# mmp/pbrt-v4

Hardware: AMD Instinct MI355X
Metric: Msamples/sec (whole node), 1920x1080 at fixed spp (higher is better)
Workload: dtype f32; 1 GPU; San Miguel 1080p 256spp (BASELINE.json configs[2]) on the sanmiguel-like stand-in at the SURVEY 8(d) spec: 10001008 unique triangles in 2000 meshes, 60 % of them in 200 object-instance definitions (two-level BVH), 10 % alpha-cut, 1k^2 image textures, diffuse / coated diffuse / dielectric / conductor, sun + 2k^2 image sky + 500 emitters, maxdepth 5, zsobol; step = 1 sample index x 1920x1080; spp=321, samples_per_pass=64, partition=single GPU

## Files before the change

### pbrt-v4_amd/csrc/common/wf_kernels.h

```cpp
#pragma once

#include "wf_bxdf.h"
#include "wf_camera.h"
#include "wf_lights.h"
#include "wf_media.h"
#include "wf_bssrdf.h"
#include "wf_hair.h"
#include "wf_measured.h"

namespace wf {

struct alignas(16) F4 { float x, y, z, w; };
struct alignas(16) I4 { int32_t x, y, z, w; };
struct alignas(8) I2 { int32_t x, y; };
WF_HD F4 toF4(S4 s) { return F4{s[0], s[1], s[2], s[3]}; }
WF_HD S4 toS4(F4 f) { return S4{{f.x, f.y, f.z, f.w}}; }

enum {
    CNT_RAY0 = 0, CNT_RAY1 = 1, CNT_ESCAPED = 2, CNT_HITLIGHT = 3, CNT_SHADOW = 4, CNT_MAT0 = 5,
    CNT_MEDIUM_SAMPLE = CNT_MAT0 + WF_MAT_NTYPES, CNT_MEDIUM_SCATTER, CNT_MIX, CNT_RETRACE, CNT_BSSRDF, CNT_SSS, CNT_CURSOR, CNT_TR0, CNT_TR1,
    CNT_RETRACE_HEAD, CNT_WAVES_DONE,
    CNT_CURSOR_SHADOW,
    CNT_MEDIUM_ROUTE,
    CNT_DEFER, CNT_DEFER_SHADOW,
    CNT_CURSOR_MEDIUM,
    CNT_COUNT
};
constexpr int CNT_STRIDE = 64;
static_assert(CNT_COUNT <= 32, "k_reset takes the counters to zero as a 32-bit mask");
enum { RAYFLAG_SPECULAR_BOUNCE = 1, RAYFLAG_ANY_NONSPECULAR = 2 };

struct RayQueueV {
    F4 *o;
    F4 *d;
    F4 *beta, *r_u, *r_l;
    F4 *ctx0;
    F4 *ctx1;
    F4 *ctx2;
    I4 *meta;
};
struct ShadowQueueV {
    F4 *o;
    F4 *d;
    F4 *Ld, *r_u, *r_l;
    int32_t *medium;
};
struct BssrdfItem {
    F4 beta, r_u;
    V3 p; float etaScale;
    V3 wo; int depth;
    N3 n; int pixelIndex;
    N3 ns; int material;
    V3 dpdus; int mediumInside;
    V2 uv; int mediumOutside; int pad;
};
struct SubsurfaceItem {
    V3 p0, p1;
    int depth, material;
    TabulatedBSSRDF bssrdf;
    F4 beta, r_u;
    float reservoirPDF;
    P3i pi;
    N3 n, ns;
    V3 dpdu, dpdv, dpdus, dpdvs;
    int mediumInside, mediumOutside;
    float etaScale;
    int pixelIndex;
};
struct WorkState {
    int maxQueueSize;
    int pixelsPerPass, samplesPerPass;
    int slotStride = 0;
    int drainEpoch = 0;
    int stripRank, stripCount, stripHeight, localRows;
    float *filterWeight;
    I2 *pPixel;
    F4 *lambda, *lambdaPdf, *L, *cameraRayWeight;
    F4 *samples0;
// ... 1525 lines not shown
```

### pbrt-v4_amd/csrc/hip/wf_backend.hip

```cpp
#include <hip/hip_runtime.h>
#include <climits>
#include <cstdio>
#include <cstring>
#include <algorithm>
#include <map>
#include <string>
#include <type_traits>
#include <utility>
#include <vector>

#pragma clang attribute push(__attribute__((uninitialized)), apply_to = variable(is_local))
#include "../common/wf_kernels.h"
#include "../common/wf_kat.h"
#pragma clang attribute pop
#include "wf_traverse.h"
#include "wf_plan.h"
#include "wf_film_develop.h"

using namespace wf;
using namespace wf::planning;

#define HIPCHK(call)                                                                                        \
    do {                                                                                                    \
        hipError_t e_ = (call);                                                                             \
        if (e_ != hipSuccess) return fail((int)e_, "%s failed: %s (%s:%d)", #call, hipGetErrorString(e_), __FILE__, __LINE__); \
    } while (0)

constexpr int BLOCK = 256;
constexpr int MAX_GRID = 256 * 8;

struct SpillArea { int *base; int rows; int *dbg; };

using ClosestWalkFn = void (*)(const SceneView, WorkState, FastBVH, int, SpillArea, int *, int, const int *);
using ShadowWalkFn = void (*)(const SceneView, WorkState, FastBVH, SpillArea, int *, int, const int *);
using TrTraceFn = void (*)(const SceneView, WorkState, FastBVH, int, SpillArea);
using TraceClosestFn = void (*)(const SceneView, FastBVH, int, const float *, wf_hit_record *, SpillArea);
using TraceAnyFn = void (*)(const SceneView, FastBVH, int, const float *, int32_t *, SpillArea);
struct WalkKernels {
    ClosestWalkFn closest = nullptr;
    ShadowWalkFn shadow = nullptr;
    ClosestWalkFn closestGen = nullptr;
    ShadowWalkFn shadowGen = nullptr;
    int grid = 1024, gridShadow = 1024, gridGen = 1024, gridShadowGen = 1024;
    TrTraceFn trTrace = nullptr;
    TraceClosestFn traceClosest = nullptr;
    TraceAnyFn traceAny = nullptr;
    TraceClosestFn traceClosest8 = nullptr;
    TraceAnyFn traceAny8 = nullptr;
};


struct wf_ctx {
    int device = 0;
    hipStream_t stream = nullptr;
    std::vector<void *> allocs;
    SceneView svHost{};
    const SceneView *svDev = nullptr;
    WorkState ws{};
    int maxQueueSize = 0;
    int *stackSpill = nullptr;
    int *dbgWords = nullptr;
    SpillArea spillArea() const { return SpillArea{stackSpill, plan.spillRows, dbgWords}; }
    FastBVH fast{};
    hipStream_t stream2 = nullptr;
    hipEvent_t evFork = nullptr, evJoin = nullptr;
    bool retracePending = false, deferJoin = false;
    hipStream_t stream3 = nullptr;
    hipEvent_t evShadowFork = nullptr, evShadowJoin = nullptr;
    int frameOverlap = 1;
    bool shadowPending = false;
    int *stackSpill2 = nullptr;
    int32_t *deferQShadow = nullptr;
    bool samplesShaded = true;
    bool cursorDirty[2] = {false, false};
    ScenePlan plan;
    WalkKernels walk;
    struct TrScratch {
        F4 *o = nullptr, *d = nullptr, *lambdaPdf = nullptr;
        float *pathTime = nullptr;
        F4 *trO = nullptr, *trD = nullptr, *trT = nullptr, *trRu = nullptr, *trRl = nullptr, *hit = nullptr;
        I4 *trRng = nullptr;
        int32_t *trQ[2] = {nullptr, nullptr}, *hitInst = nullptr;
        int32_t *counters = nullptr;
        size_t capacity = 0;
        struct Slot { void **p; size_t elem; bool wavefront; };
        std::vector<Slot> slots() {
            return {{(void **)&o, sizeof(F4), false}, {(void **)&d, sizeof(F4), false}, {(void **)&lambdaPdf, sizeof(F4), false}, {(void **)&pathTime, sizeof(float), false},
                    {(void **)&trO, sizeof(F4), true}, {(void **)&trD, sizeof(F4), true}, {(void **)&trT, sizeof(F4), true}, {(void **)&trRu, sizeof(F4), true},
                    {(void **)&trRl, sizeof(F4), true}, {(void **)&hit, sizeof(F4), true}, {(void **)&trRng, sizeof(I4), true},
                    {(void **)&trQ[0], sizeof(int32_t), true}, {(void **)&trQ[1], sizeof(int32_t), true}, {(void **)&hitInst, sizeof(int32_t), true}};
        }
    } trScratch;
    int32_t *probeCursor = nullptr;
// ... 480 lines not shown
        }
        const bool valid = idx < n;
        RayWalk w;
        w.node = NODE_NONE;
        w.prim = -1;
        w.route = 0;
        w.tMax = 0;
        w.b0 = w.b1 = w.b2 = 0;
        w.inst = w.curInst = -1;
        if (valid) {
            V3 o, d;
            float tMax;
            fetch(idx, &o, &d, &tMax);
            WalkInit(bvh, w, o, d, tMax);
            if constexpr (INST || GEN > 0) StoreWorldRay(o, d);
            st.reset();
        }
        while (__any(w.node != NODE_NONE)) {
            while (WalkDescend<INST, ANY>(w)) {
                if (w.node >= 0) {
                    U4 nd[QNODE_U4];
                    FetchNode(bvh, w.node, nd);
                    InteriorStep<!ANY>(bvh, w, st, nd);
                }
            }
            LeafPhase<ANY, GEN, INST>(sv, bvh, w, st, fetch, idx);
        }
        if constexpr (!ANY && RetraceInline(GenBase(GEN))) {
            static_assert(ANY || !GenDefer(GEN), "the inline re-walk's `w.route = rh.route` would drop WALK_DEFER: the handing-over variants must walk with BatchTraceRefill");
            if (valid && WalkAmbiguous(w)) {
                V3 o, d;
                float t0;
                fetch(idx, &o, &d, &t0);
                const float tB = __builtin_fminf(2 * WalkBound(bvh, WalkT(w)) - WalkT(w), t0);
                const RefHit rh = RetraceRefOrder<GenBase(GEN), GenAnim(GEN)>(bvh.sv, o.x, o.y, o.z, d.x, d.y, d.z, tB, st.spill, st.spillStride, st.rows, st.dbg, GenAnim(GEN) ? g_time[threadIdx.x] : 0.f);
                w.prim = rh.prim; w.inst = rh.inst; w.route = rh.route;
                w.tMax = rh.t; w.b0 = rh.b0; w.b1 = rh.b1; w.b2 = rh.b2;
            }
        }
        finish(idx, valid, w);
    }
}

#ifndef WF_REFILL_AT
#define WF_REFILL_AT 40
#endif
#ifndef WF_GUIDED_CHUNK
#define WF_GUIDED_CHUNK 6
#endif
#ifndef WF_GUIDED_DIV
#define WF_GUIDED_DIV 4
#endif
template <bool ANY, int GEN, bool INST = false, bool DRAIN = false, typename Fetch, typename Finish>
__device__ inline void BatchTraceRefill(const SceneView &sv, const FastBVH &bvh, int n, LdsStackT &st, Fetch fetch, Finish finish, int *cursor = nullptr, int chunk = 4,
                                        int workBlocks = 0) {
    if (workBlocks <= 0) workBlocks = (int)gridDim.x;
    if (n < 2 * workBlocks * TBLOCK) cursor = nullptr;
    if (cursor && st.dbg && threadIdx.x == 0 && blockIdx.x == 0) atomicOr(st.dbg + 3, 1);
    const int lane = threadIdx.x & 63;
    const int waveId = (blockIdx.x * TBLOCK + threadIdx.x) >> 6, nWaves = (workBlocks * TBLOCK) >> 6;
    const int runRays = cursor ? 64 * chunk : 64;
    int next = 0, end = 0, staticJ = 0;
    int lastB = 0;
    bool exhausted = false;
    int idx = -1;
#if WF_WALK_ZERO
    RayWalk w{};
#else
    RayWalk w;
#endif
    w.node = NODE_NONE;
    w.prim = -1;
    w.route = 0;
    w.tMax = 0;
    w.b0 = w.b1 = w.b2 = 0;
    w.inst = w.curInst = -1;
    WalkStats ws_;
    auto retire = [&]() {
        finish(idx, true, w);
        idx = -1;
    };
    while (true) {
        const unsigned long long act = __ballot(w.node != NODE_NONE);
        const int nAct = __popcll(act);
        if (nAct <= WF_REFILL_AT && !exhausted) {
            const bool idle = w.node == NODE_NONE;
            if (idle && idx >= 0) retire();
            const int need = 64 - nAct;
            const int rank = __popcll(~act & ((1ull << lane) - 1ull));
            int served = 0;
            while (served < need) {
                if (next >= end) {
                    int b;
                    int rr = runRays;
                    if (cursor) {
#if WF_GUIDED_CHUNK
                        if constexpr (ANY && GenBase(GEN) <= 1) { int c = (n - lastB) / (nWaves * 64 * WF_GUIDED_DIV); c = c < 1 ? 1 : (c > WF_GUIDED_CHUNK ? WF_GUIDED_CHUNK : c); rr = 64 * c; }
#endif
                        b = 0;
                        if (lane == 0) b = atomicAdd(cursor, rr);
                        b = __builtin_amdgcn_readfirstlane(b);
                        lastB = b < n ? b : n;
                    } else {
                        b = (staticJ * nWaves + waveId) * 64;
                        ++staticJ;
                    }
                    next = b;
                    end = b + rr < n ? b + rr : n;
                    if (next >= n) { exhausted = true; break; }
                }
                const int take = need - served < end - next ? need - served : end - next;
                if (idle && rank >= served && rank < served + take) idx = next + (rank - served);
                next += take;
                served += take;
            }
            ws_.add(3, idle && idx >= 0);
            if (idle && idx >= 0) {
                V3 o, d;
                float tMax;
                fetch(idx, &o, &d, &tMax);
                WalkInit(bvh, w, o, d, tMax);
                if constexpr (INST || GEN > 0) StoreWorldRay(o, d);
                st.reset();
            }
            if (exhausted && !__any(w.node != NODE_NONE)) break;
        } else if (nAct == 0) break;
        while (WalkDescend<INST, ANY>(w)) {
            ws_.add(0, w.node >= 0);
            if (w.node >= 0) {
                U4 nd[QNODE_U4];
                FetchNode(bvh, w.node, nd);
                InteriorStep<!ANY>(bvh, w, st, nd);
            }
        }
        if constexpr (WF_WALK_STATS != 0) ws_.add(1, w.node < 0 && w.node != NODE_NONE && !(INST && AtTransition(w.node)));
        const int ranT = LeafPhase<ANY, GEN, INST>(sv, bvh, w, st, fetch, idx);
        if constexpr (WF_WALK_STATS != 0) { if (ranT) { ws_.c[4] += 1; ws_.c[5] += (unsigned long long)ranT; } }
    }
    ws_.flush(st.dbg, ANY ? 1 : 0);
    if (idx >= 0) retire();
}
template <bool ANY, int GEN, bool INST, bool DRAIN = false, typename Fetch, typename Finish>
__device__ inline void TraceQueue(const SceneView &sv, const FastBVH &bvh, int n, LdsStackT &st, Fetch fetch, Finish finish, int *cursor = nullptr, int chunk = 4,
                                  int workBlocks = 0) {
    if constexpr (ANY || DRAIN || !RetraceInline(GenBase(GEN))) BatchTraceRefill<ANY, GEN, INST, DRAIN>(sv, bvh, n, st, fetch, finish, cursor, chunk, workBlocks);
    else BatchTrace<ANY, GEN, INST>(sv, bvh, n, st, fetch, finish, cursor, chunk);
}
#ifndef WF_SERVICE_BLOCKS
#define WF_SERVICE_BLOCKS 16
#endif
__device__ inline int ServiceBlocks() { return (int)gridDim.x >= 8 * WF_SERVICE_BLOCKS ? WF_SERVICE_BLOCKS : 0; }
template <int GEN, bool INST, bool ANIM = false>
__device__ inline void DrainRetrace(const SceneView &sv, const WorkState &ws, const FastBVH &bvh, int cur, LdsStackT &st, bool service) {
    int *cnt = ws.counters + CNT_RETRACE * CNT_STRIDE, *head = ws.counters + CNT_RETRACE_HEAD * CNT_STRIDE, *done = ws.counters + CNT_WAVES_DONE * CNT_STRIDE;
    const int lane = threadIdx.x & 63;
    const int totalWaves = (int)gridDim.x * (TBLOCK / 64), workerWaves = ((int)gridDim.x - ServiceBlocks()) * (TBLOCK / 64);
    const RayQueueV &q = ws.rq[cur];
    auto takeSome = [&]() -> bool {
        int base = 0, take = 0;
        if (lane == 0) {
            while (true) {
                const int h = __hip_atomic_load(head, __ATOMIC_RELAXED, __HIP_MEMORY_SCOPE_AGENT), c = __hip_atomic_load(cnt, __ATOMIC_RELAXED, __HIP_MEMORY_SCOPE_AGENT);
                if (h >= c) break;
                const int t = c - h < 64 ? c - h : 64;
                if (atomicCAS(head, h, h + t) == h) { base = h; take = t; break; }
            }
        }
        base = __builtin_amdgcn_readfirstlane(base);
        take = __builtin_amdgcn_readfirstlane(take);
        if (take == 0) return false;
        if (lane < take) {
            unsigned long long e;
            while ((uint32_t)((e = __hip_atomic_load(&ws.retraceQ64[base + lane], __ATOMIC_ACQUIRE, __HIP_MEMORY_SCOPE_AGENT)) >> 32) != (uint32_t)ws.drainEpoch) {}
            const int i = (int)(uint32_t)(e & 0xffffffffull);
            const float tB = BitsToFloat((uint32_t)__hip_atomic_load(&ws.retraceQ[base + lane], __ATOMIC_RELAXED, __HIP_MEMORY_SCOPE_AGENT));
            const F4 o = q.o[i], d = q.d[i];
            RefHit rh;
            int tries = 0;
            do { rh = RetraceRefOrder<GEN, ANIM>(bvh.sv, o.x, o.y, o.z, d.x, d.y, d.z, tB, st.spill, st.spillStride, st.rows, st.dbg, o.w); } while (rh.prim < 0 && ++tries < 4);
            if (st.dbg && tries) { atomicAdd(st.dbg + 5, tries); if (rh.prim < 0) atomicOr(st.dbg + 6, 1); }
            if (st.dbg) {
                const bool badIndex = i < 0 || i >= ws.counters[(CNT_RAY0 + cur) * CNT_STRIDE];
                const bool badHit = rh.prim >= 0 && !(rh.t <= tB);
                const bool badTag = (uint32_t)(__hip_atomic_load(&ws.retraceQ64[base + lane], __ATOMIC_RELAXED, __HIP_MEMORY_SCOPE_AGENT) >> 32) != (uint32_t)ws.drainEpoch;
                if (badIndex || badHit || badTag) atomicOr(st.dbg + 6, 2);
            }
            ws.routeCode[i] = rh.route;
            ws.hit[i] = F4{BitsToFloat((uint32_t)rh.prim), rh.b0, rh.b1, rh.b2};
            if (INST) ws.hitInst[i] = rh.prim >= 0 ? rh.inst : -1;
            if (sv.haveMedia) ws.hitT[i] = rh.prim >= 0 ? rh.t : WF_INFINITY;
        }
        return true;
    };
    auto signOff = [&]() -> int {
        int prev = 0;
        if (lane == 0) { __threadfence(); prev = atomicAdd(done, 1); }
        return __builtin_amdgcn_readfirstlane(prev);
    };
    bool last;
    if (!service) {
        while (takeSome()) {}
        last = signOff() == totalWaves - 1;
        if (last) while (takeSome()) {}
    } else {
        while (true) {
            if (takeSome()) continue;
            int dn = 0;
            if (lane == 0) dn = __hip_atomic_load(done, __ATOMIC_RELAXED, __HIP_MEMORY_SCOPE_AGENT);
            dn = __builtin_amdgcn_readfirstlane(dn);
            if (dn >= workerWaves) {
                if (takeSome()) continue;
                break;
            }
            __builtin_amdgcn_s_sleep(64);
        }
        last = signOff() == totalWaves - 1;
    }
    if (last && lane == 0) {
        __hip_atomic_store(head, 0, __ATOMIC_RELAXED, __HIP_MEMORY_SCOPE_AGENT);
        __hip_atomic_store(cnt, 0, __ATOMIC_RELAXED, __HIP_MEMORY_SCOPE_AGENT);
        __hip_atomic_store(done, 0, __ATOMIC_RELAXED, __HIP_MEMORY_SCOPE_AGENT);
    }
}

constexpr uint32_t ROUTE_SKIP = 0x80000000u;
constexpr int TWavesFor(int gen, int triangleWaves) { return gen == 3 ? 2 : triangleWaves; }
template <int GENX, bool INST = false>
__global__ void __launch_bounds__(TBLOCK, TWavesFor(GenBase(GENX), INST ? WF_TWAVES_INST : WF_TWAVES_CLOSEST)) k_closest_fast(const SceneView svArg, WorkState ws, FastBVH bvh, int cur, SpillArea sp, int *cursor = nullptr, int chunk = 4, const int *list = nullptr) {
    constexpr int GEN = GenBase(GENX);
    const SceneView &sv = SvOf<false>(svArg);
    const int n = list ? ws.counters[(CNT_DEFER) * CNT_STRIDE] : ws.counters[(CNT_RAY0 + cur) * CNT_STRIDE];
    const int gtid = blockIdx.x * TBLOCK + threadIdx.x, stride = gridDim.x * TBLOCK;
    LdsStackT st{sp.base + gtid, stride, 0, 0, sp.rows, sp.dbg};
    const RayQueueV q = ws.rq[cur];
    constexpr bool DRAIN = RetraceInline(GEN);
    const int workBlocks = DRAIN ? (int)gridDim.x - ServiceBlocks() : (int)gridDim.x;
    if (DRAIN && (int)blockIdx.x >= workBlocks) { DrainRetrace<GEN, INST, GenAnim(GENX)>(sv, ws, bvh, cur, st, true); return; }
    TraceQueue<false, GENX, INST, DRAIN>(
        sv, bvh, n, st,
        [&](int i0, V3 *o, V3 *d, float *tMax) {
            const int i = list ? list[i0] : i0;
            F4 o4 = q.o[i], d4 = q.d[i];
            *o = V3{o4.x, o4.y, o4.z}; *d = V3{d4.x, d4.y, d4.z}; *tMax = WF_INFINITY;
            if constexpr (GenAnim(GENX)) {
                g_time[threadIdx.x] = o4.w;
                ws.pathTime[q.meta[i].x] = o4.w;
            }
        },
        [&](int i0, bool valid, const RayWalk &w) {
            const int i = (list && valid) ? list[i0] : i0;
            if constexpr (GenDefer(GENX))
                if (valid && (w.route & WALK_DEFER)) {
                    ws.deferQ[QueueAlloc(&ws.counters[(CNT_DEFER) * CNT_STRIDE])] = i;
                    ws.routeCode[i] = ROUTE_SKIP;
                    return;
                }
            const bool amb = valid && WalkAmbiguous(w);
            if (amb) {
                const int slot = atomicAdd(&ws.counters[(CNT_RETRACE) * CNT_STRIDE], 1);
                const float bound = 2 * WalkBound(bvh, WalkT(w)) - WalkT(w);
                if constexpr (DRAIN) {
                    if (sp.dbg) atomicAdd(sp.dbg + 4, 1);
                    __hip_atomic_store(&ws.retraceQ[slot], (int)FloatToBits(bound), __ATOMIC_RELAXED, __HIP_MEMORY_SCOPE_AGENT);
                    __hip_atomic_store(&ws.retraceQ64[slot], (unsigned long long)(uint32_t)i | ((unsigned long long)(uint32_t)ws.drainEpoch << 32), __ATOMIC_RELEASE, __HIP_MEMORY_SCOPE_AGENT);
                    return;
                } else {
                    ws.retraceQ[slot] = i;
                    ws.hit[i] = F4{0, bound, 0, 0};
                }
            }
            if (!valid) return;
            ws.routeCode[i] = amb ? ROUTE_SKIP : (uint32_t)w.route;
            if (amb) return;
            ws.hit[i] = F4{BitsToFloat((uint32_t)w.prim), w.b0, w.b1, w.b2};
            if (INST) ws.hitInst[i] = w.prim >= 0 ? w.inst : -1;
            if (sv.haveMedia) ws.hitT[i] = w.prim >= 0 ? WalkT(w) : WF_INFINITY;
        }, cursor, chunk, workBlocks);
    if constexpr (DRAIN) DrainRetrace<GEN, INST, GenAnim(GENX)>(sv, ws, bvh, cur, st, false);
}
constexpr int RBLOCK = 1024;
constexpr int RouteBlock(bool anim) { return anim ? BLOCK : RBLOCK; }
template <bool GENERAL, bool ANIM = false>
__global__ void __launch_bounds__(RouteBlock(ANIM)) k_route_hits(const SceneView svArg, WorkState ws, int cur) {
    constexpr int RB = RouteBlock(ANIM);
    const SceneView &sv = SvOf<true>(svArg);
    const int n = ws.counters[(CNT_RAY0 + cur) * CNT_STRIDE];
    for (int base = blockIdx.x * RB; base < n; base += gridDim.x * RB) {
        const int i = base + threadIdx.x;
        bool valid = i < n;
        uint32_t route = 0;
        F4 h{0, 0, 0, 0};
        int inst = -1;
        float tHit = 0;
        if (valid) {
            route = ws.routeCode[i];
            if (route & ROUTE_SKIP) valid = false;
            else {
                h = ws.hit[i];
                if (sv.nInstances > 0) inst = ws.hitInst[i];
                if (sv.haveMedia) tHit = ws.hitT[i];
            }
        }
        KRouteHitBlock<GENERAL, ANIM>(sv, ws, cur, i, valid, (int)FloatToBits(h.x), route, tHit, h.y, h.z, h.w, inst);
    }
}
__global__ void __launch_bounds__(BLOCK) k_closest_retrace(const SceneView sv, WorkState ws, int cur, int *stackSpill) {
    const int n = ws.counters[(CNT_RETRACE) * CNT_STRIDE];
    const int gtid = blockIdx.x * BLOCK + threadIdx.x, stride = gridDim.x * BLOCK;
    LdsStack st{stackSpill + gtid, stride, 0};
    for (int qi = gtid; qi < n; qi += stride) {
        const int i = ws.retraceQ[qi];
        F4 o = ws.rq[cur].o[i], d = ws.rq[cur].d[i];
        ClosestHit ch;
        st.n = 0;
        bool found = BVHIntersectClosest(sv, V3{o.x, o.y, o.z}, V3{d.x, d.y, d.z}, ws.hit[i].y, st, &ch);
        KAfterClosestHit(sv, ws, cur, i, found, ch.prim, ch.inst, ch.h.t, ch.h.b0, ch.h.b1, ch.h.b2);
    }
}
__global__ void __launch_bounds__(BLOCK) k_subsurface_probe(const SceneView sv, WorkState ws) {
    const int n = ws.counters[(CNT_BSSRDF) * CNT_STRIDE];
    for (int i = blockIdx.x * BLOCK + threadIdx.x; i < n; i += gridDim.x * BLOCK) KSubsurfaceProbe(sv, ws, i);
}
template <bool ANIM>
__global__ void __launch_bounds__(BLOCK) k_intersect_one_random(const SceneView sv, WorkState ws, int *stackSpill) {
    const int n = ws.counters[(CNT_SSS) * CNT_STRIDE];
    const int gtid = blockIdx.x * BLOCK + threadIdx.x, stride = gridDim.x * BLOCK;
    LdsStack st{stackSpill + gtid, stride, 0};
    for (int i = gtid; i < n; i += stride) KIntersectOneRandom<ANIM>(sv, ws, i, st);
}
template <bool ANIM>
__global__ void __launch_bounds__(BLOCK) k_trace_one_random(const SceneView sv, int n, const float *segs, int segStride, const int32_t *material, const float *times,
// ... 458 lines not shown

struct ClosestWalk { using Fn = ClosestWalkFn; template <int G, bool I> static Fn of() { return k_closest_fast<G, I>; } };
struct ShadowWalk { using Fn = ShadowWalkFn; template <int G, bool I> static Fn of() { return k_shadow_fast<G, I>; } };
struct TrTraceWalk { using Fn = TrTraceFn; template <int G, bool I> static Fn of() { return k_tr_trace<G, I>; } };
struct TraceClosestWalk { using Fn = TraceClosestFn; template <int G, bool I> static Fn of() { return k_trace_closest_fast<G, I>; } };
struct TraceAnyWalk { using Fn = TraceAnyFn; template <int G, bool I> static Fn of() { return k_trace_any_fast<G, I>; } };
struct TraceClosestWalk8 { using Fn = TraceClosestFn; template <int G, bool I> static Fn of() { return k_trace_closest_fast<G, I, 8>; } };
struct TraceAnyWalk8 { using Fn = TraceAnyFn; template <int G, bool I> static Fn of() { return k_trace_any_fast<G, I, 8>; } };
template <typename K, bool INST, int G>
static typename K::Fn WalkVariant() {
    if constexpr (GenAnim(G) && !INST) return nullptr;
    else return K::template of<G, INST>();
}
template <typename K, int... G>
static typename K::Fn PickWalk(int genx, bool inst, std::integer_sequence<int, G...>) {
    typename K::Fn f = nullptr;
    ((genx == G ? (void)(f = inst ? WalkVariant<K, true, G>() : WalkVariant<K, false, G>()) : (void)0), ...);
    return f;
}
static int PickWalkKernels(wf_ctx *ctx) {
    using QueueWalks = std::integer_sequence<int, 0, 1, 2, 3, GenX(0, true, false), GenX(1, true, false), GenX(0, false, true), GenX(1, false, true)>;
    const bool inst = ctx->svHost.nInstances > 0;
    const int gen = ctx->plan.genMode;
    const int first = ctx->plan.deferGeneral ? GenX(ctx->plan.genTri, true, false) : GenX(gen, false, ctx->plan.animFast);
    WalkKernels k;
    k.closest = PickWalk<ClosestWalk>(first, inst, QueueWalks{});
    k.shadow = PickWalk<ShadowWalk>(first, inst, QueueWalks{});
    if (ctx->plan.deferGeneral) {
        k.closestGen = PickWalk<ClosestWalk>(gen, inst, QueueWalks{});
        k.shadowGen = PickWalk<ShadowWalk>(gen, inst, QueueWalks{});
    }
    k.traceClosest = PickWalk<TraceClosestWalk>(gen, inst, std::integer_sequence<int, 0, 1, 2, 3>{});
    k.traceAny = PickWalk<TraceAnyWalk>(gen, inst, std::integer_sequence<int, 0, 1, 2, 3>{});
    {
        using TimedWalks = std::integer_sequence<int, 0, 1, 2, 3, GenX(0, false, true), GenX(1, false, true)>;
        k.traceClosest8 = PickWalk<TraceClosestWalk8>(GenX(gen, false, ctx->plan.animFast), inst, TimedWalks{});
        k.traceAny8 = PickWalk<TraceAnyWalk8>(GenX(gen, false, ctx->plan.animFast), inst, TimedWalks{});
    }
    if (RetraceInline(gen)) k.trTrace = PickWalk<TrTraceWalk>(GenX(gen, false, ctx->plan.animFast), inst, std::integer_sequence<int, 0, 1, GenX(0, false, true), GenX(1, false, true)>{});
    if (!k.closest || !k.shadow || !k.traceClosest || !k.traceAny || !k.traceClosest8 || !k.traceAny8 || (ctx->plan.deferGeneral && (!k.closestGen || !k.shadowGen)) || (RetraceInline(gen) && !k.trTrace))
        return fail(-1, "no walk kernel for this scene (genMode %d, genTri %d, two-class %d, animated %d, instances %d)", gen, ctx->plan.genTri, (int)ctx->plan.deferGeneral, (int)ctx->plan.animFast, (int)inst);
    hipDeviceProp_t prop;
    HIPCHK(hipGetDeviceProperties(&prop, ctx->device));
    const int maxG = MAX_GRID * BLOCK / TBLOCK;
    auto residentGrid = [&](auto kernel, int *out) {
        int perCU = 0;
        HIPCHK(hipOccupancyMaxActiveBlocksPerMultiprocessor(&perCU, (const void *)kernel, TBLOCK, 0));
        *out = std::min(maxG, std::max(1, perCU) * prop.multiProcessorCount);
        return 0;
    };
    int e;
    if ((e = residentGrid(k.closest, &k.grid)) || (e = residentGrid(k.shadow, &k.gridShadow))) return e;
    if (ctx->plan.deferGeneral && ((e = residentGrid(k.closestGen, &k.gridGen)) || (e = residentGrid(k.shadowGen, &k.gridShadowGen)))) return e;
    ctx->walk = k;
    return 0;
}

extern "C" {

int wf_abi_version(void) { return WF_ABI_VERSION; }

constexpr int SCRATCH_PRIME_WORDS = 896;
__global__ void k_scratch_prime(int *out, int n) {
    volatile int buf[SCRATCH_PRIME_WORDS];
    for (int i = 0; i < n; ++i) buf[(i * 131) % SCRATCH_PRIME_WORDS] = i;
    out[threadIdx.x] = buf[(n * 7) % SCRATCH_PRIME_WORDS];
}
static void DestroyCtx(wf_ctx *ctx) {
    (void)hipSetDevice(ctx->device);
    if (ctx->stream) (void)hipStreamSynchronize(ctx->stream);
    if (ctx->stream3) (void)hipStreamSynchronize(ctx->stream3);
    for (void *p : ctx->allocs) (void)hipFree(p);
    for (const wf_ctx::TrScratch::Slot &sl : ctx->trScratch.slots())
        if (*sl.p) (void)hipFree(*sl.p);
    if (ctx->trScratch.counters) (void)hipFree(ctx->trScratch.counters);
    for (auto &e : ctx->events) { (void)hipEventDestroy(e.a); (void)hipEventDestroy(e.b); }
    for (auto e : ctx->eventPool) (void)hipEventDestroy(e);
    if (ctx->stream) (void)hipStreamDestroy(ctx->stream);
    if (ctx->stream2) (void)hipStreamDestroy(ctx->stream2);
    if (ctx->stream3) (void)hipStreamDestroy(ctx->stream3);
    if (ctx->evShadowFork) (void)hipEventDestroy(ctx->evShadowFork);
    if (ctx->evShadowJoin) (void)hipEventDestroy(ctx->evShadowJoin);
    if (ctx->evFork) (void)hipEventDestroy(ctx->evFork);
    if (ctx->evJoin) (void)hipEventDestroy(ctx->evJoin);
    delete ctx;
}
static int InitCtx(wf_ctx *c, const Switches &sw) {
    HIPCHK(hipStreamCreateWithFlags(&c->stream, hipStreamNonBlocking));
    HIPCHK(hipStreamCreateWithFlags(&c->stream2, hipStreamNonBlocking));
    HIPCHK(hipStreamCreateWithFlags(&c->stream3, hipStreamNonBlocking));
    HIPCHK(hipEventCreateWithFlags(&c->evFork, hipEventDisableTiming));
    HIPCHK(hipEventCreateWithFlags(&c->evJoin, hipEventDisableTiming));
    HIPCHK(hipEventCreateWithFlags(&c->evShadowFork, hipEventDisableTiming));
    HIPCHK(hipEventCreateWithFlags(&c->evShadowJoin, hipEventDisableTiming));
    c->frameOverlap = sw.frameOverlap;
    c->samplesShaded = sw.samplesShaded;
    c->traceLaunch = sw.traceLaunch;
    if (sw.scratchPrime) {
        DeviceScratch tmp(c->stream);
        int *out = nullptr;
        if (int e = tmp.alloc(&out, (size_t)64)) return e;
        hipLaunchKernelGGL(k_scratch_prime, dim3(1), dim3(64), 0, c->stream, out, 8);
        hipLaunchKernelGGL(k_scratch_prime, dim3(1), dim3(64), 0, c->stream2, out, 8);
        hipLaunchKernelGGL(k_scratch_prime, dim3(1), dim3(64), 0, c->stream3, out, 8);
        HIPCHK(hipStreamSynchronize(c->stream));
        HIPCHK(hipStreamSynchronize(c->stream2));
        HIPCHK(hipStreamSynchronize(c->stream3));
    }
    return 0;
}
int wf_ctx_create(int device, wf_ctx **out) {
    if (!out) return fail(-1, "null out");
    int ndev = 0;
    HIPCHK(hipGetDeviceCount(&ndev));
    if (ndev <= 0) return fail(-1, "no HIP device visible: libwfhip has no CPU fallback");
    if (device < 0 || device >= ndev) return fail(-1, "device %d out of range (0..%d)", device, ndev - 1);
    HIPCHK(hipSetDevice(device));
    wf_ctx *c = new wf_ctx();
    c->device = device;
    if (int e = InitCtx(c, Switches::FromEnv())) { DestroyCtx(c); return e; }
    *out = c;
    return 0;
}

int wf_ctx_destroy(wf_ctx *ctx) {
    if (ctx) DestroyCtx(ctx);
    return 0;
}

int wf_sync(wf_ctx *ctx) {
    if (!ctx) return fail(-1, "null context");
    useDevice(ctx);
    HIPCHK(hipStreamSynchronize(ctx->stream));
    HIPCHK(hipGetLastError());
    if (ctx->dbgWords) {
        int overflow = 0;
        HIPCHK(hipMemcpy(&overflow, ctx->dbgWords + 1, sizeof(int), hipMemcpyDeviceToHost));
        if (overflow) return fail(-1, "traversal stack overflow: a walk needed more than %d + %d node-stack entries (results are incomplete)", TSTACK, ctx->plan.spillRows);
        int unresolved = 0;
        HIPCHK(hipMemcpy(&unresolved, ctx->dbgWords + 6, sizeof(int), hipMemcpyDeviceToHost));
        if (unresolved & 1) return fail(-1, "a near-tie re-walk found no hit where the production walk had one (results are incomplete)");
        if (unresolved & 2) return fail(-1, "a near-tie queue entry failed its validation (ray index, bound or launch tag): results are incomplete");
        int fatal = 0;
        HIPCHK(hipMemcpy(&fatal, ctx->dbgWords + 7, sizeof(int), hipMemcpyDeviceToHost));
        if (fatal) return fail(-1, "%s", FatalMessage(fatal));
        if (getenv("WF_DEBUG_DRAIN")) {
            int h[8];
            HIPCHK(hipMemcpy(h, ctx->dbgWords, sizeof(h), hipMemcpyDeviceToHost));
            fprintf(stderr, "[drain] spilled %d, re-walks %d, pushes %d, repeated re-walks %d, unresolved %d\n", h[0], h[2], h[4], h[5], h[6]);
#if WF_WALK_STATS
            unsigned long long c[16];
            HIPCHK(hipMemcpy(c, ctx->dbgWords + 8, sizeof(c), hipMemcpyDeviceToHost));
            const char *ph[4] = {"interior", "leaf", "transition", "refill"};
            for (int k = 0; k < 2; ++k)
                for (int q = 0; q < 4; ++q)
                    fprintf(stderr, "[walk stats] %s %-26s wave iterations %llu, lanes %llu (%.1f per iteration)\n", k ? "any-hit" : "closest", ph[q], c[k * 8 + 2 * q], c[k * 8 + 2 * q + 1],
                            c[k * 8 + 2 * q] ? (double)c[k * 8 + 2 * q + 1] / (double)c[k * 8 + 2 * q] : 0.0);
#endif
        }
    }
    return 0;
}
int wf_debug_counters(wf_ctx *ctx, uint64_t out[4], int reset) {
    if (!ctx || !ctx->sceneLoaded || !out) return fail(-1, "wf_debug_counters: no scene uploaded");
    int h[4] = {0, 0, 0, 0};
    HIPCHK(hipStreamSynchronize(ctx->stream));
    HIPCHK(hipMemcpy(h, ctx->dbgWords, sizeof(h), hipMemcpyDeviceToHost));
    for (int i = 0; i < 4; ++i) out[i] = (uint64_t)(unsigned)h[i];
    if (reset) HIPCHK(hipMemset(ctx->dbgWords, 0, sizeof(h)));
    return 0;
}
void *wf_stream(wf_ctx *ctx) { return ctx ? (void *)ctx->stream : nullptr; }

static int UploadTables(wf_ctx *ctx, const wf_scene_desc *d, const Switches &sw) {
    SceneView &sv = ctx->svHost;
    const ScenePlan &plan = ctx->plan;
    int e = 0;
    if ((e = devUpload(ctx, &sv.P, d->P, (size_t)3 * d->n_vertices))) return e;
    if ((e = devUpload(ctx, &sv.N, d->N, (size_t)3 * d->n_vertices))) return e;
    if ((e = devUpload(ctx, &sv.UV, d->UV, (size_t)2 * d->n_vertices))) return e;
    if (d->n_tangents > 0 && (e = devUpload(ctx, &sv.S, d->S, (size_t)3 * d->n_tangents))) return e;
    if ((e = devUpload(ctx, &sv.triIndices, d->tri_indices, (size_t)3 * d->n_triangles))) return e;
    if ((e = devUpload(ctx, &sv.triMesh, d->tri_mesh, (size_t)d->n_triangles + d->n_quadrics))) return e;
    sv.shadeTris = nullptr;
    if (d->n_triangles > 0 && sw.shadeTris) {
        std::vector<ShadeTri> st((size_t)d->n_triangles);
        for (size_t t = 0; t < (size_t)d->n_triangles; ++t) {
            const int32_t *ix = d->tri_indices + 3 * t;
            const int flags = d->meshes[d->tri_mesh[t]].flags;
            ShadeTri r{};
            for (int k = 0; k < 3; ++k) {
                for (int a = 0; a < 3; ++a) r.p[3 * k + a] = d->P[3 * (size_t)ix[k] + a];
                if ((flags & WF_MESH_HAS_N) && d->N) for (int a = 0; a < 3; ++a) r.n[3 * k + a] = d->N[3 * (size_t)ix[k] + a];
                if ((flags & WF_MESH_HAS_UV) && d->UV) for (int a = 0; a < 2; ++a) r.uv[2 * k + a] = d->UV[2 * (size_t)ix[k] + a];
            }
// ... 269 lines not shown
        int planes = 0;
        for (int m = 1; m < WF_MAT_NTYPES; ++m) if (ctx->plan.matPresent[m]) planes = std::max(planes, NeePlanes(m));
        if (planes > 0 && (e = devAlloc(ctx, &ws.neeRec, n * (size_t)planes))) return e;
    }
    if ((e = devAlloc(ctx, &ws.routeCode, n))) return e;
    ctx->maxQueueSize = max_queue_size;
    ctx->queuesAllocated = true;
    return 0;
}

int wf_set_pass_samples(wf_ctx *ctx, int sample_step, int n_samples) {
    if (int e = checkReady(ctx)) return e;
    if (n_samples < 1 || n_samples > ctx->ws.samplesPerPass) return fail(-1, "n_samples %d outside 1..%d", n_samples, ctx->ws.samplesPerPass);
    if (sample_step < 1) return fail(-1, "sample_step must be >= 1");
    ctx->passStep = sample_step;
    ctx->passSamples = n_samples;
    ctx->ws.slotStride = ctx->pixelMajor ? n_samples : 0;
    return 0;
}

int wf_set_strips(wf_ctx *ctx, int rank, int count, int height, int *local_rows) {
    if (!ctx || !ctx->sceneLoaded) return fail(-1, "no scene uploaded");
    useDevice(ctx);
    if (count < 1 || rank < 0 || rank >= count || height < 1) return fail(-1, "wf_set_strips: rank %d of %d, height %d", rank, count, height);
    int rows = 0;
    for (int y = 0; y < ctx->H; ++y) rows += (y / height) % count == rank;
    ctx->ws.stripRank = rank; ctx->ws.stripCount = count; ctx->ws.stripHeight = height; ctx->ws.localRows = count > 1 ? rows : ctx->H;
    if (local_rows) *local_rows = ctx->ws.localRows;
    return 0;
}

int wf_film_clear(wf_ctx *ctx) {
    if (!ctx || !ctx->sceneLoaded) return fail(-1, "no scene uploaded");
    useDevice(ctx);
    HIPCHK(hipMemsetAsync(ctx->ws.film, 0, (size_t)ctx->W * ctx->H * 4 * sizeof(double), ctx->stream));
    if (ctx->ws.filmGBuffer) HIPCHK(hipMemsetAsync(ctx->ws.filmGBuffer, 0, (size_t)ctx->W * ctx->H * sizeof(wf_gbuffer_pixel), ctx->stream));
    if (ctx->ws.filmSpectral) HIPCHK(hipMemsetAsync(ctx->ws.filmSpectral, 0, (size_t)ctx->W * ctx->H * 2 * ctx->svHost.film.n_buckets * sizeof(double), ctx->stream));
    HIPCHK(hipMemsetAsync(ctx->ws.stats, 0, (129 + 16) * sizeof(unsigned long long), ctx->stream));
    HIPCHK(hipMemsetAsync(ctx->ws.trav, 0, 8 * sizeof(unsigned long long), ctx->stream));
    return 0;
}

int wf_reset_ray_queue(wf_ctx *ctx, int which) {
    if (int e = checkReady(ctx)) return e;
    LAUNCH("Reset ray queue", k_reset, 1, ctx->ws, 1u << (CNT_RAY0 + (which & 1)), -1, 0);
    return 0;
}
int wf_reset_stage_queues(wf_ctx *ctx, int depth) {
    if (int e = checkReady(ctx)) return e;
    const int cur = depth & 1;
    constexpr unsigned matBits = ((1u << WF_MAT_NTYPES) - 1u) << CNT_MAT0;
    constexpr unsigned stageMask = (1u << CNT_ESCAPED) | (1u << CNT_HITLIGHT) | matBits |
        (1u << CNT_MEDIUM_SAMPLE) | (1u << CNT_MEDIUM_SCATTER) | (1u << CNT_MIX) | (1u << CNT_RETRACE) | (1u << CNT_BSSRDF) | (1u << CNT_SSS) |
        (1u << CNT_RETRACE_HEAD) | (1u << CNT_WAVES_DONE) | (1u << CNT_CURSOR) | (1u << CNT_MEDIUM_ROUTE) | (1u << CNT_DEFER) | (1u << CNT_CURSOR_MEDIUM);
    static_assert((stageMask & ((1u << CNT_SHADOW) | (1u << CNT_CURSOR_SHADOW) | (1u << CNT_DEFER_SHADOW))) == 0 && CNT_SHADOW != CNT_RAY0 && CNT_SHADOW != CNT_RAY1,
                  "the stage reset must not zero a counter of the shadow stage, which may be running beside it");
    const unsigned mask = stageMask | (1u << (CNT_RAY0 + (cur ^ 1)));
    LAUNCH("Reset queues before tracing rays", k_reset, 1, ctx->ws, mask, 1 + statDepth(depth), CNT_RAY0 + cur);
    ctx->cursorDirty[0] = false;
    return 0;
}
int wf_gen_camera_rays(wf_ctx *ctx, int y0, int sample_index) {
    if (int e = checkReady(ctx)) return e;
    ctx->passY0 = y0;
    if (ctx->ws.sampleTops) LAUNCH("Sampler index prefixes", k_sample_tops, gridFor(5 * ctx->ws.pixelsPerPass), ctx->svHost, ctx->ws, y0, 0);
    if (ctx->svHost.camera.type == WF_CAMERA_REALISTIC)
        LAUNCH("Reset ray queue", k_reset, 1, ctx->ws, 1u << CNT_RAY0, -1, 0);
    LAUNCH("Generate camera rays", (ctx->svHost.camera.anim.actually_animated ? k_gen_camera_rays<true> : k_gen_camera_rays<false>), gridFor(ctx->maxQueueSize), ctx->svHost, ctx->ws, y0, sample_index,
           ctx->passStep, ctx->passSamples);
    LAUNCH("Update camera ray stats", k_reset, 1, ctx->ws, 0u, 0, CNT_RAY0);
    return 0;
}
int wf_gen_ray_samples(wf_ctx *ctx, int depth, int sample_index) {
    if (int e = checkReady(ctx)) return e;
    const bool tops = ctx->ws.sampleTops != nullptr && ctx->passY0 != INT_MIN;
    if (tops) LAUNCH("Sampler index prefixes", k_sample_tops, gridFor(5 * ctx->ws.pixelsPerPass), ctx->svHost, ctx->ws, ctx->passY0, 6 + 7 * depth);
    LAUNCH("Generate ray samples - ZSobolSampler", k_gen_ray_samples, gridFor(ctx->maxQueueSize), ctx->svHost, ctx->ws, depth & 1, sample_index, ctx->passStep,
           tops ? depth : -1);
    return 0;
}
static int JoinRetrace(wf_ctx *ctx) {
    if (!ctx->retracePending) return 0;
    HIPCHK(hipStreamWaitEvent(ctx->stream, ctx->evJoin, 0));
    ctx->retracePending = false;
    return 0;
}
int wf_intersect_closest(wf_ctx *ctx, int depth) {
    if (int e = checkReady(ctx)) return e;
    const bool anim = ctx->svHost.haveAnimated;
    if (ctx->countTraversal)
        LAUNCH("Intersect closest", (anim ? k_intersect_closest<true, true> : k_intersect_closest<true, false>), gridFor(ctx->maxQueueSize), ctx->svHost, ctx->ws, depth & 1, ctx->stackSpill);
    else if (ctx->plan.fastOk) {
        const WalkKernels &k = ctx->walk;
        int *cursor = ctx->ws.counters + CNT_CURSOR * CNT_STRIDE;
        if (ctx->cursorDirty[0]) HIPCHK(hipMemsetAsync(cursor, 0, sizeof(int), ctx->stream));
        ctx->cursorDirty[0] = true;
        ctx->ws.drainEpoch = (ctx->ws.drainEpoch + 1) & 0x7fffffff;
        if (ctx->ws.drainEpoch == 0) ctx->ws.drainEpoch = 1;
        if (k.closestGen) {
            FastBVH triFast = ctx->fast;
            triFast.absBand = triFast.absBandTri; triFast.tieRel = triFast.tieRelTri;
            LAUNCHT("Intersect closest", k.closest, k.grid, ctx->svHost, ctx->ws, triFast, depth & 1, ctx->spillArea(), cursor, ctx->plan.cursorChunk, (const int *)nullptr);
            LAUNCHT("Intersect closest: rays that met a general primitive", k.closestGen, k.gridGen, ctx->svHost, ctx->ws, ctx->fast, depth & 1, ctx->spillArea(), (int *)nullptr, ctx->plan.cursorChunk, (const int *)ctx->ws.deferQ);
        } else
            LAUNCHT("Intersect closest", k.closest, k.grid, ctx->svHost, ctx->ws, ctx->fast, depth & 1, ctx->spillArea(), cursor, ctx->plan.cursorChunk, (const int *)nullptr);
        const bool overlap = !RetraceInline(ctx->plan.genMode) && ctx->profile != 1 && !ctx->traceLaunch;
        if (overlap) {
            HIPCHK(hipEventRecord(ctx->evFork, ctx->stream));
            HIPCHK(hipStreamWaitEvent(ctx->stream2, ctx->evFork, 0));
            hipLaunchKernelGGL(k_closest_retrace, dim3(128), dim3(BLOCK), 0, ctx->stream2, ctx->svHost, ctx->ws, depth & 1, ctx->stackSpill);
            HIPCHK(hipEventRecord(ctx->evJoin, ctx->stream2));
            ctx->retracePending = true;
        }
        {
            Prof prof_(ctx, "Route hits");
            const int g = std::min(MAX_GRID, std::max(1, (ctx->maxQueueSize + RBLOCK - 1) / RBLOCK));
            if (anim)
                hipLaunchKernelGGL((k_route_hits<true, true>), dim3(std::min(MAX_GRID, std::max(1, (ctx->maxQueueSize + BLOCK - 1) / BLOCK))), dim3(BLOCK), 0, ctx->stream, ctx->svHost, ctx->ws, depth & 1);
            else if (ctx->plan.genMode > 1 || ctx->svHost.nInstances > 0) hipLaunchKernelGGL(k_route_hits<true>, dim3(g), dim3(RBLOCK), 0, ctx->stream, ctx->svHost, ctx->ws, depth & 1);
            else hipLaunchKernelGGL(k_route_hits<false>, dim3(g), dim3(RBLOCK), 0, ctx->stream, ctx->svHost, ctx->ws, depth & 1);
        }
        if (ctx->retracePending) {
            if (ctx->deferJoin) return 0;
            if (int e = JoinRetrace(ctx)) return e;
        } else if (!RetraceInline(ctx->plan.genMode))
            LAUNCH("Intersect closest: near-tie re-trace", k_closest_retrace, 128, ctx->svHost, ctx->ws, depth & 1, ctx->stackSpill);
        if (ctx->svHost.haveMix) LAUNCH("Resolve MixMaterial hits", (anim ? k_resolve_mix<true> : k_resolve_mix<false>), gridFor(ctx->maxQueueSize), ctx->svHost, ctx->ws, depth & 1);
    } else
        LAUNCH("Intersect closest", (anim ? k_intersect_closest<false, true> : k_intersect_closest<false, false>), gridFor(ctx->maxQueueSize), ctx->svHost, ctx->ws, depth & 1, ctx->stackSpill);
    return 0;
}
int wf_medium_sample(wf_ctx *ctx, int depth) {
    if (int e = checkReady(ctx)) return e;
    if (!ctx->svHost.haveMedia) return 0;
    LAUNCH("Sample medium interaction", (ctx->plan.mediumLean ? k_medium_sample<true> : k_medium_sample<false>), gridFor(ctx->maxQueueSize), ctx->svHost, ctx->ws, depth & 1);
    LAUNCH("Sample medium interaction: route surface hits", (ctx->svHost.haveAnimated ? k_medium_route<true> : k_medium_route<false>), gridFor(ctx->maxQueueSize), ctx->svHost, ctx->ws, depth & 1);
    if (depth == ctx->maxDepth) return 0;
    LAUNCH("Sample direct/indirect - Henyey-Greenstein", (ctx->plan.rareLights ? k_medium_scatter<true> : k_medium_scatter<false>), gridFor(ctx->maxQueueSize), ctx->svHost, ctx->ws, depth & 1);
    return 0;
}
using TrSegmentFn = void (*)(const SceneView, WorkState, int);
static TrSegmentFn TrSegmentKernel(const wf_ctx *ctx) {
    if (ctx->plan.animFast) return ctx->plan.mediumLean ? k_tr_segment<true, true> : k_tr_segment<false, true>;
    return ctx->plan.mediumLean ? k_tr_segment<true> : k_tr_segment<false>;
}
int wf_intersect_shadow_tr(wf_ctx *ctx, int depth) {
    if (int e = checkReady(ctx)) return e;
    if (!ctx->svHost.haveMedia) return fail(-1, "wf_intersect_shadow_tr: the scene has no media (use wf_intersect_shadow)");
    const int route = ctx->countTraversal ? 0 : ctx->plan.trRoute;
    if (route == 2) {
        LAUNCH("Reset transmittance queues", k_reset, 1, ctx->ws, (1u << CNT_TR0) | (1u << CNT_TR1), -1, 0);
        LAUNCH("Intersect shadow (Tr): begin", k_tr_begin, gridFor(ctx->maxQueueSize), ctx->svHost, ctx->ws);
        for (int seg = 0; seg < WF_TR_SEGMENTS; ++seg) {
            const int cur = seg & 1;
            LAUNCHT("Intersect shadow (Tr): trace", ctx->walk.trTrace, ctx->walk.grid, ctx->svHost, ctx->ws, ctx->fast, cur, ctx->spillArea());
            LAUNCH("Intersect shadow (Tr): segment", TrSegmentKernel(ctx), gridFor(ctx->maxQueueSize), ctx->svHost, ctx->ws, cur);
            LAUNCH("Reset transmittance queues", k_reset, 1, ctx->ws, 1u << (CNT_TR0 + cur), -1, 0);
        }
// ... 824 lines not shown
```

Baseline: 450.7 Msamples/s.

## Split near-tie retrace service into a separate kernel on a second stream

The near-tie retrace service blocks move out of the closest-hit walk kernel into their own kernel, launched on a second stream beside a walk grid shrunk by the service block count. Worker waves now only sign off when done. Service waves poll the retrace queue until every worker has signed off, then reset the counters. A wall-clock timeout with a fatal flag guards against deadlock if the two kernels are not co-resident. The aim is to drop the per-block branching and last-wave drain in the walk kernel and let the walk run with its own occupancy, at the cost of depending on concurrent scheduling of the two kernels.

```diff
diff --git a/pbrt-v4_amd/csrc/common/wf_kernels.h b/pbrt-v4_amd/csrc/common/wf_kernels.h
--- a/pbrt-v4_amd/csrc/common/wf_kernels.h
+++ b/pbrt-v4_amd/csrc/common/wf_kernels.h
@@ -23,7 +23,7 @@
     CNT_CURSOR_SHADOW,
     CNT_MEDIUM_ROUTE,
     CNT_DEFER, CNT_DEFER_SHADOW,
-    CNT_CURSOR_MEDIUM,
+    CNT_SERVICE_DONE,
     CNT_COUNT
 };
 constexpr int CNT_STRIDE = 64;
diff --git a/pbrt-v4_amd/csrc/hip/wf_backend.hip b/pbrt-v4_amd/csrc/hip/wf_backend.hip
--- a/pbrt-v4_amd/csrc/hip/wf_backend.hip
+++ b/pbrt-v4_amd/csrc/hip/wf_backend.hip
@@ -32,6 +32,7 @@
 struct SpillArea { int *base; int rows; int *dbg; };
 
 using ClosestWalkFn = void (*)(const SceneView, WorkState, FastBVH, int, SpillArea, int *, int, const int *);
+using ClosestServiceFn = void (*)(const SceneView, WorkState, FastBVH, int, SpillArea, int, int);
 using ShadowWalkFn = void (*)(const SceneView, WorkState, FastBVH, SpillArea, int *, int, const int *);
 using TrTraceFn = void (*)(const SceneView, WorkState, FastBVH, int, SpillArea);
 using TraceClosestFn = void (*)(const SceneView, FastBVH, int, const float *, wf_hit_record *, SpillArea);
@@ -39,6 +40,8 @@
 struct WalkKernels {
     ClosestWalkFn closest = nullptr;
     ShadowWalkFn shadow = nullptr;
+    ClosestServiceFn service = nullptr;
+    int gridService = 0;
     ClosestWalkFn closestGen = nullptr;
     ShadowWalkFn shadowGen = nullptr;
     int grid = 1024, gridShadow = 1024, gridGen = 1024, gridShadowGen = 1024;
@@ -625,13 +628,11 @@
 #define WF_GUIDED_DIV 4
 #endif
 template <bool ANY, int GEN, bool INST = false, bool DRAIN = false, typename Fetch, typename Finish>
-__device__ inline void BatchTraceRefill(const SceneView &sv, const FastBVH &bvh, int n, LdsStackT &st, Fetch fetch, Finish finish, int *cursor = nullptr, int chunk = 4,
-                                        int workBlocks = 0) {
-    if (workBlocks <= 0) workBlocks = (int)gridDim.x;
-    if (n < 2 * workBlocks * TBLOCK) cursor = nullptr;
+__device__ inline void BatchTraceRefill(const SceneView &sv, const FastBVH &bvh, int n, LdsStackT &st, Fetch fetch, Finish finish, int *cursor = nullptr, int chunk = 4) {
+    if (n < 2 * (int)gridDim.x * TBLOCK) cursor = nullptr;
     if (cursor && st.dbg && threadIdx.x == 0 && blockIdx.x == 0) atomicOr(st.dbg + 3, 1);
     const int lane = threadIdx.x & 63;
-    const int waveId = (blockIdx.x * TBLOCK + threadIdx.x) >> 6, nWaves = (workBlocks * TBLOCK) >> 6;
+    const int waveId = (blockIdx.x * TBLOCK + threadIdx.x) >> 6, nWaves = ((int)gridDim.x * TBLOCK) >> 6;
     const int runRays = cursor ? 64 * chunk : 64;
     int next = 0, end = 0, staticJ = 0;
     int lastB = 0;
@@ -714,20 +715,24 @@
     if (idx >= 0) retire();
 }
 template <bool ANY, int GEN, bool INST, bool DRAIN = false, typename Fetch, typename Finish>
-__device__ inline void TraceQueue(const SceneView &sv, const FastBVH &bvh, int n, LdsStackT &st, Fetch fetch, Finish finish, int *cursor = nullptr, int chunk = 4,
-                                  int workBlocks = 0) {
-    if constexpr (ANY || DRAIN || !RetraceInline(GenBase(GEN))) BatchTraceRefill<ANY, GEN, INST, DRAIN>(sv, bvh, n, st, fetch, finish, cursor, chunk, workBlocks);
+__device__ inline void TraceQueue(const SceneView &sv, const FastBVH &bvh, int n, LdsStackT &st, Fetch fetch, Finish finish, int *cursor = nullptr, int chunk = 4) {
+    if constexpr (ANY || DRAIN || !RetraceInline(GenBase(GEN))) BatchTraceRefill<ANY, GEN, INST, DRAIN>(sv, bvh, n, st, fetch, finish, cursor, chunk);
     else BatchTrace<ANY, GEN, INST>(sv, bvh, n, st, fetch, finish, cursor, chunk);
 }
 #ifndef WF_SERVICE_BLOCKS
 #define WF_SERVICE_BLOCKS 16
 #endif
-__device__ inline int ServiceBlocks() { return (int)gridDim.x >= 8 * WF_SERVICE_BLOCKS ? WF_SERVICE_BLOCKS : 0; }
+constexpr long long SERVICE_GIVE_UP_TICKS = 20ll * 100000000ll;
+__device__ inline void WorkerSignOff(const WorkState &ws) {
+    __threadfence();
+    if ((threadIdx.x & 63) == 0) atomicAdd(ws.counters + CNT_WAVES_DONE * CNT_STRIDE, 1);
+}
 template <int GEN, bool INST, bool ANIM = false>
-__device__ inline void DrainRetrace(const SceneView &sv, const WorkState &ws, const FastBVH &bvh, int cur, LdsStackT &st, bool service) {
+__device__ inline void ServeRetrace(const SceneView &sv, const WorkState &ws, const FastBVH &bvh, int cur, LdsStackT &st, int workerWaves) {
     int *cnt = ws.counters + CNT_RETRACE * CNT_STRIDE, *head = ws.counters + CNT_RETRACE_HEAD * CNT_STRIDE, *done = ws.counters + CNT_WAVES_DONE * CNT_STRIDE;
+    int *served = ws.counters + CNT_SERVICE_DONE * CNT_STRIDE;
     const int lane = threadIdx.x & 63;
-    const int totalWaves = (int)gridDim.x * (TBLOCK / 64), workerWaves = ((int)gridDim.x - ServiceBlocks()) * (TBLOCK / 64);
+    const int serviceWaves = (int)gridDim.x * (TBLOCK / 64);
     const RayQueueV &q = ws.rq[cur];
     auto takeSome = [&]() -> bool {
         int base = 0, take = 0;
@@ -765,34 +770,31 @@
         }
         return true;
     };
-    auto signOff = [&]() -> int {
-        int prev = 0;
-        if (lane == 0) { __threadfence(); prev = atomicAdd(done, 1); }
-        return __builtin_amdgcn_readfirstlane(prev);
-    };
-    bool last;
-    if (!service) {
-        while (takeSome()) {}
-        last = signOff() == totalWaves - 1;
-        if (last) while (takeSome()) {}
-    } else {
-        while (true) {
+    long long idleSince = wall_clock64();
+    int seen = -1;
+    while (true) {
+        if (takeSome()) { idleSince = wall_clock64(); continue; }
+        int dn = 0;
+        if (lane == 0) dn = __hip_atomic_load(done, __ATOMIC_RELAXED, __HIP_MEMORY_SCOPE_AGENT);
+        dn = __builtin_amdgcn_readfirstlane(dn);
+        if (dn >= workerWaves) {
             if (takeSome()) continue;
-            int dn = 0;
-            if (lane == 0) dn = __hip_atomic_load(done, __ATOMIC_RELAXED, __HIP_MEMORY_SCOPE_AGENT);
-            dn = __builtin_amdgcn_readfirstlane(dn);
-            if (dn >= workerWaves) {
-                if (takeSome()) continue;
-                break;
-            }
-            __builtin_amdgcn_s_sleep(64);
-        }
-        last = signOff() == totalWaves - 1;
-    }
-    if (last && lane == 0) {
+            break;
+        }
+        if (dn != seen) { seen = dn; idleSince = wall_clock64(); }
+        else if (wall_clock64() - idleSince > SERVICE_GIVE_UP_TICKS) {
+            if (lane == 0 && st.dbg) atomicOr(st.dbg + 6, 4);
+            break;
+        }
+        __builtin_amdgcn_s_sleep(64);
+    }
+    int prev = 0;
+    if (lane == 0) { __threadfence(); prev = atomicAdd(served, 1); }
+    if (__builtin_amdgcn_readfirstlane(prev) == serviceWaves - 1 && lane == 0) {
         __hip_atomic_store(head, 0, __ATOMIC_RELAXED, __HIP_MEMORY_SCOPE_AGENT);
         __hip_atomic_store(cnt, 0, __ATOMIC_RELAXED, __HIP_MEMORY_SCOPE_AGENT);
         __hip_atomic_store(done, 0, __ATOMIC_RELAXED, __HIP_MEMORY_SCOPE_AGENT);
+        __hip_atomic_store(served, 0, __ATOMIC_RELAXED, __HIP_MEMORY_SCOPE_AGENT);
     }
 }
 
@@ -807,8 +809,6 @@
     LdsStackT st{sp.base + gtid, stride, 0, 0, sp.rows, sp.dbg};
     const RayQueueV q = ws.rq[cur];
     constexpr bool DRAIN = RetraceInline(GEN);
-    const int workBlocks = DRAIN ? (int)gridDim.x - ServiceBlocks() : (int)gridDim.x;
-    if (DRAIN && (int)blockIdx.x >= workBlocks) { DrainRetrace<GEN, INST, GenAnim(GENX)>(sv, ws, bvh, cur, st, true); return; }
     TraceQueue<false, GENX, INST, DRAIN>(
         sv, bvh, n, st,
         [&](int i0, V3 *o, V3 *d, float *tMax) {
@@ -848,8 +848,15 @@
             ws.hit[i] = F4{BitsToFloat((uint32_t)w.prim), w.b0, w.b1, w.b2};
             if (INST) ws.hitInst[i] = w.prim >= 0 ? w.inst : -1;
             if (sv.haveMedia) ws.hitT[i] = w.prim >= 0 ? WalkT(w) : WF_INFINITY;
-        }, cursor, chunk, workBlocks);
-    if constexpr (DRAIN) DrainRetrace<GEN, INST, GenAnim(GENX)>(sv, ws, bvh, cur, st, false);
+        }, cursor, chunk);
+    if constexpr (DRAIN) WorkerSignOff(ws);
+}
+template <int GEN, bool INST, bool ANIM>
+__global__ void __launch_bounds__(TBLOCK, ANIM ? 3 : 4) k_closest_service(const SceneView svArg, WorkState ws, FastBVH bvh, int cur, SpillArea sp, int walkGrid, int workerWaves) {
+    const SceneView &sv = SvOf<false>(svArg);
+    const int gtid = blockIdx.x * TBLOCK + threadIdx.x, stride = gridDim.x * TBLOCK;
+    LdsStackT st{sp.base + (size_t)sp.rows * walkGrid * TBLOCK + gtid, stride, 0, 0, sp.rows, sp.dbg};
+    ServeRetrace<GEN, INST, ANIM>(sv, ws, bvh, cur, st, workerWaves);
 }
 constexpr int RBLOCK = 1024;
 constexpr int RouteBlock(bool anim) { return anim ? BLOCK : RBLOCK; }
@@ -1414,6 +1421,13 @@
     int e;
     if ((e = residentGrid(k.closest, &k.grid)) || (e = residentGrid(k.shadow, &k.gridShadow))) return e;
     if (ctx->plan.deferGeneral && ((e = residentGrid(k.closestGen, &k.gridGen)) || (e = residentGrid(k.shadowGen, &k.gridShadowGen)))) return e;
+    if (RetraceInline(GenBase(first))) {
+        const bool anim = GenAnim(first);
+        if (GenBase(first) == 0) k.service = !inst ? k_closest_service<0, false, false> : anim ? k_closest_service<0, true, true> : k_closest_service<0, true, false>;
+        else k.service = !inst ? k_closest_service<1, false, false> : anim ? k_closest_service<1, true, true> : k_closest_service<1, true, false>;
+        if (k.grid < 2) return fail(-1, "the closest-hit walk's resident grid (%d) leaves no workgroup for its near-tie service", k.grid);
+        k.gridService = std::min(WF_SERVICE_BLOCKS, std::max(1, k.grid / 8));
+    }
     ctx->walk = k;
     return 0;
 }
@@ -1503,6 +1517,7 @@
         HIPCHK(hipMemcpy(&unresolved, ctx->dbgWords + 6, sizeof(int), hipMemcpyDeviceToHost));
         if (unresolved & 1) return fail(-1, "a near-tie re-walk found no hit where the production walk had one (results are incomplete)");
         if (unresolved & 2) return fail(-1, "a near-tie queue entry failed its validation (ray index, bound or launch tag): results are incomplete");
+        if (unresolved & 4) return fail(-1, "the near-tie service gave up waiting for its closest-hit walk to sign off (results are incomplete)");
         int fatal = 0;
         HIPCHK(hipMemcpy(&fatal, ctx->dbgWords + 7, sizeof(int), hipMemcpyDeviceToHost));
         if (fatal) return fail(-1, "%s", FatalMessage(fatal));
@@ -1878,7 +1893,7 @@
     constexpr unsigned matBits = ((1u << WF_MAT_NTYPES) - 1u) << CNT_MAT0;
     constexpr unsigned stageMask = (1u << CNT_ESCAPED) | (1u << CNT_HITLIGHT) | matBits |
         (1u << CNT_MEDIUM_SAMPLE) | (1u << CNT_MEDIUM_SCATTER) | (1u << CNT_MIX) | (1u << CNT_RETRACE) | (1u << CNT_BSSRDF) | (1u << CNT_SSS) |
-        (1u << CNT_RETRACE_HEAD) | (1u << CNT_WAVES_DONE) | (1u << CNT_CURSOR) | (1u << CNT_MEDIUM_ROUTE) | (1u << CNT_DEFER) | (1u << CNT_CURSOR_MEDIUM);
+        (1u << CNT_RETRACE_HEAD) | (1u << CNT_WAVES_DONE) | (1u << CNT_CURSOR) | (1u << CNT_MEDIUM_ROUTE) | (1u << CNT_DEFER) | (1u << CNT_SERVICE_DONE);
     static_assert((stageMask & ((1u << CNT_SHADOW) | (1u << CNT_CURSOR_SHADOW) | (1u << CNT_DEFER_SHADOW))) == 0 && CNT_SHADOW != CNT_RAY0 && CNT_SHADOW != CNT_RAY1,
                   "the stage reset must not zero a counter of the shadow stage, which may be running beside it");
     const unsigned mask = stageMask | (1u << (CNT_RAY0 + (cur ^ 1)));
@@ -1909,6 +1924,25 @@
     if (!ctx->retracePending) return 0;
     HIPCHK(hipStreamWaitEvent(ctx->stream, ctx->evJoin, 0));
     ctx->retracePending = false;
+    return 0;
+}
+static int LaunchClosestWalk(wf_ctx *ctx, const FastBVH &fast, int cur, int *cursor) {
+    const WalkKernels &k = ctx->walk;
+    if (!k.service) {
+        LAUNCHT("Intersect closest", k.closest, k.grid, ctx->svHost, ctx->ws, fast, cur, ctx->spillArea(), cursor, ctx->plan.cursorChunk, (const int *)nullptr);
+        return 0;
+    }
+    const int walkGrid = k.grid - k.gridService, workerWaves = walkGrid * (TBLOCK / 64);
+    const bool aside = ctx->profile != 1 && !ctx->traceLaunch;
+    if (aside) HIPCHK(hipEventRecord(ctx->evFork, ctx->stream));
+    LAUNCHT("Intersect closest", k.closest, walkGrid, ctx->svHost, ctx->ws, fast, cur, ctx->spillArea(), cursor, ctx->plan.cursorChunk, (const int *)nullptr);
+    if (aside) {
+        HIPCHK(hipStreamWaitEvent(ctx->stream2, ctx->evFork, 0));
+        LAUNCHT_ON(ctx->stream2, "Intersect closest: near-tie service", k.service, k.gridService, ctx->svHost, ctx->ws, fast, cur, ctx->spillArea(), walkGrid, workerWaves);
+        HIPCHK(hipEventRecord(ctx->evJoin, ctx->stream2));
+        HIPCHK(hipStreamWaitEvent(ctx->stream, ctx->evJoin, 0));
+    } else
+        LAUNCHT("Intersect closest: near-tie service", k.service, k.gridService, ctx->svHost, ctx->ws, fast, cur, ctx->spillArea(), walkGrid, workerWaves);
     return 0;
 }
 int wf_intersect_closest(wf_ctx *ctx, int depth) {
@@ -1926,10 +1960,9 @@
         if (k.closestGen) {
             FastBVH triFast = ctx->fast;
             triFast.absBand = triFast.absBandTri; triFast.tieRel = triFast.tieRelTri;
-            LAUNCHT("Intersect closest", k.closest, k.grid, ctx->svHost, ctx->ws, triFast, depth & 1, ctx->spillArea(), cursor, ctx->plan.cursorChunk, (const int *)nullptr);
+            if (int e = LaunchClosestWalk(ctx, triFast, depth & 1, cursor)) return e;
             LAUNCHT("Intersect closest: rays that met a general primitive", k.closestGen, k.gridGen, ctx->svHost, ctx->ws, ctx->fast, depth & 1, ctx->spillArea(), (int *)nullptr, ctx->plan.cursorChunk, (const int *)ctx->ws.deferQ);
-        } else
-            LAUNCHT("Intersect closest", k.closest, k.grid, ctx->svHost, ctx->ws, ctx->fast, depth & 1, ctx->spillArea(), cursor, ctx->plan.cursorChunk, (const int *)nullptr);
+        } else if (int e = LaunchClosestWalk(ctx, ctx->fast, depth & 1, cursor)) return e;
         const bool overlap = !RetraceInline(ctx->plan.genMode) && ctx->profile != 1 && !ctx->traceLaunch;
         if (overlap) {
             HIPCHK(hipEventRecord(ctx->evFork, ctx->stream));
```

Result: slower. 434.7 Msamples/s (-3.5%).
